# openclimatefix/graph_weather

Measured on AMD Instinct MI355X. Metric: forward forecasts/sec (1° grid, 102→78 feat), higher is better.
Workload: dtype f32; 1 GPU; c2: GraphWeatherForecaster 1deg grid (64800 nodes), 102->78 feat, batch=2 on rank 0, fp32, mesh res 2 (5882 nodes), random-init weights; global_batch=2, parallelism=batch-sharded x1, no collective in forward

## Files before the change

### graph_weather_amd/_lib.py

```python
from __future__ import annotations

import ctypes
import os
import subprocess
from ctypes import POINTER, Structure, c_char_p, c_float, c_int, c_int32, c_int64, c_size_t, c_void_p

_HERE = os.path.dirname(os.path.abspath(__file__))
CSRC = os.path.join(_HERE, "csrc")
LIB_PATH = os.path.join(CSRC, "libgw_amd.so")
HIPCC_FLAGS = ["--offload-arch=gfx950", "-O3", "-std=c++17", "-munsafe-fp-atomics", "-shared", "-fPIC"]

ABI_VERSION = 19
DTYPE_F32, DTYPE_BF16, DTYPE_BF16X3 = 0, 1, 2
LAYOUT_ROWS_F32, LAYOUT_EDGE_TILES_BF16, LAYOUT_ROWS_F16, LAYOUT_ROWS_BF16K = 0, 1, 2, 3
EDGE_DETERMINISTIC, EDGE_SEGMENT_TILES, EDGE_AGG_BF16K, EDGE_SEGMENT_SPLIT = 1, 2, 4, 8

EXPORTS = [
    "gw_version", "gw_last_error", "gw_debug_timestamps", "gw_packed_floats", "gw_pack_linear", "gw_packed_bytes_bf16",
    "gw_pack_linear_bf16", "gw_packed_bytes_bf16x3", "gw_pack_linear_bf16x3", "gw_padded_n", "gw_pad_vector", "gw_pack_many", "gw_mlp_chain_backward", "gw_mlp_chain_backward_bf16x3", "gw_mlp_ln_chain_backward",
    "gw_mlp_forward", "gw_mlp_post_forward", "gw_project_forward", "gw_edge_update_forward", "gw_edge_update_workspace_bytes", "gw_edge_tiles_bytes",
    "gw_edge_rows_to_tiles", "gw_node_update_forward", "gw_node_update_row_split_groups", "gw_node_update_head_forward",
    "gw_normalized_mse_forward", "gw_gemm_f32", "gw_relu_backward", "gw_layernorm_backward", "gw_gather_rows",
    "gw_segment_sum_rows", "gw_normalized_mse_backward", "gw_adamw_step", "gw_nudging_forward", "gw_nudging_backward",
    "gw_linear_forward", "gw_linear_gather_forward", "gw_layernorm_forward", "gw_add_rows", "gw_gather_rows_wide", "gw_segment_sum_rows_wide",
    "gw_constraint_workspace_bytes", "gw_constraint_forward", "gw_constraint_backward",
    "gw_thermal_conv_forward", "gw_thermal_conv_wgrad_workspace_bytes", "gw_thermal_conv_wgrad", "gw_thermal_colsum_workspace_bytes",
    "gw_thermal_colsum", "gw_thermal_groupnorm_workspace_bytes", "gw_thermal_groupnorm_forward", "gw_thermal_groupnorm_backward",
    "gw_thermal_maxpool_forward", "gw_thermal_maxpool_backward", "gw_thermal_resize_forward", "gw_thermal_resize_backward",
    "gw_thermal_rows",
    "gw_amse_mmax", "gw_amse_dft_rows", "gw_amse_legendre_floats", "gw_amse_coeff_floats", "gw_amse_workspace_bytes",
    "gw_amse_forward", "gw_amse_backward",
    "gw_modulate_workspace_bytes", "gw_sdl_forward", "gw_sdl_backward", "gw_film_forward", "gw_film_backward",
    "gw_attention_forward", "gw_attention_backward", "gw_knn_interpolate_forward", "gw_knn_interpolate_backward",
    "gw_gelu_forward", "gw_gelu_backward",
    "gw_attention_axial_forward", "gw_attention_axial_backward",
    "gw_patch_workspace_bytes", "gw_patch_embed_forward", "gw_patch_embed_backward", "gw_patch_expand_forward",
    "gw_patch_expand_backward",
    "gw_attention_masked_forward", "gw_attention_masked_backward",
    "gw_earth_loss_workspace_bytes", "gw_earth_loss_forward", "gw_earth_loss_backward",
    "gw_token_mean_forward", "gw_token_mean_backward", "gw_relu_forward", "gw_row_scale",
    "gw_conv3d_workspace_bytes", "gw_conv3d_forward", "gw_conv3d_backward",
    "gw_gemm_tn_ordered_workspace_bytes", "gw_gemm_tn_ordered", "gw_layernorm_backward_ordered_workspace_bytes",
    "gw_layernorm_backward_ordered",
    "gw_encoder_fused_forward",
    "gw_graph_attention_forward", "gw_graph_attention_backward", "gw_cond_layernorm_forward", "gw_cond_layernorm_backward",
    "gw_beta_gate_forward", "gw_beta_gate_workspace_bytes", "gw_beta_gate_backward", "gw_silu_forward", "gw_silu_backward",
    "gw_fourier_forward", "gw_fourier_backward",
    "gw_graph_attention_batched_forward", "gw_graph_attention_batched_backward", "gw_cond_layernorm_grouped_forward",
    "gw_cond_layernorm_grouped_workspace_bytes", "gw_cond_layernorm_grouped_backward", "gw_gencast_precond_input_forward",
    "gw_gencast_precond_input_backward", "gw_gencast_precond_output_forward", "gw_gencast_precond_output_backward",
    "gw_isht_lmax", "gw_isht_legendre_floats", "gw_isht_workspace_bytes", "gw_isht_forward",
    "gw_gencast_sampler_combine", "gw_gencast_weighted_mse_workspace_bytes", "gw_gencast_weighted_mse_forward",
    "gw_gencast_weighted_mse_backward",
    "gw_cond_layernorm_fanout_forward", "gw_cond_layernorm_fanout_workspace_bytes", "gw_cond_layernorm_fanout_backward",
    "gw_linear_gather_grouped_forward", "gw_segment_sum_rows_grouped",
]

GEMM_NN, GEMM_TN, GEMM_TN_BF16X3 = 0, 1, 2


class GwOperand(Structure):
    _fields_ = [("ptr", c_void_p), ("index", c_void_p), ("rows_per_batch", c_int32), ("ld", c_int32), ("k", c_int32),
                ("projected", c_int32), ("layout", c_int32)]


class GwMlpWeights(Structure):
    _fields_ = [("w1", c_void_p * 3), ("b1", c_void_p), ("w_mid", c_void_p), ("b_mid", c_void_p), ("w_out", c_void_p),
# ... 109 lines not shown
    L.gw_pad_vector.argtypes = [c_void_p, c_int, c_void_p, c_void_p]
    L.gw_mlp_chain_backward.restype = c_int
    L.gw_mlp_chain_backward.argtypes = [c_int64, c_void_p, c_int32, c_int32, POINTER(c_void_p), POINTER(c_void_p), POINTER(c_void_p),
                                        c_int32, POINTER(c_void_p), POINTER(c_void_p), c_void_p]
    L.gw_mlp_chain_backward_bf16x3.restype = c_int
    L.gw_mlp_chain_backward_bf16x3.argtypes = L.gw_mlp_chain_backward.argtypes
    L.gw_mlp_ln_chain_backward.restype = c_int
    L.gw_mlp_ln_chain_backward.argtypes = [c_int32, c_int64, c_void_p, c_int32, c_void_p, c_int32, c_int32, c_void_p, c_int32,
                                           c_void_p, c_void_p, c_void_p, c_void_p, c_void_p,
                                           c_int32, POINTER(c_void_p), POINTER(c_void_p), POINTER(c_void_p), c_void_p,
                                           c_int32, POINTER(c_void_p), POINTER(c_void_p), POINTER(c_void_p), c_int32, ctypes.c_uint32, c_void_p]
    L.gw_pack_many.restype = c_int
    L.gw_pack_many.argtypes = [c_int32, c_int32, POINTER(GwPackItem), c_int32, POINTER(GwPadItem), c_void_p]
    L.gw_mlp_forward.restype = c_int
    L.gw_mlp_forward.argtypes = [c_int64, c_int32, POINTER(GwOperand), POINTER(GwMlpWeights), POINTER(GwOperand),
                                 c_void_p, c_int32, POINTER(GwActivationSave), c_void_p]
    L.gw_mlp_post_forward.restype = c_int
    L.gw_mlp_post_forward.argtypes = [c_int64, c_int32, POINTER(GwOperand), POINTER(GwMlpWeights), c_void_p, c_int32, c_int32,
                                      POINTER(c_void_p), POINTER(c_void_p), c_int32, c_void_p]
    L.gw_edge_update_forward.restype = c_int
    L.gw_edge_update_forward.argtypes = [c_int32, c_int32, c_void_p, c_void_p, POINTER(GwOperand), POINTER(GwOperand),
                                         POINTER(GwOperand), POINTER(GwOperand), POINTER(GwMlpWeights), c_void_p, c_int32, c_void_p,
                                         c_int32, POINTER(GwActivationSave), c_void_p, c_size_t, c_int32, c_void_p]
    L.gw_encoder_fused_forward.restype = c_int
    L.gw_encoder_fused_forward.argtypes = [c_int32, c_int32, c_void_p, c_void_p, POINTER(GwOperand), POINTER(GwMlpWeights),
                                           POINTER(GwOperand), POINTER(GwOperand), POINTER(GwOperand), POINTER(GwMlpWeights), c_void_p,
                                           c_int32, POINTER(GwActivationSave), c_int32, c_void_p]
    L.gw_edge_tiles_bytes.restype = c_size_t
    L.gw_edge_tiles_bytes.argtypes = [c_int32, c_int32]
    L.gw_edge_rows_to_tiles.restype = c_int
    L.gw_edge_rows_to_tiles.argtypes = [c_int32, c_int32, c_void_p, c_int32, c_int32, c_void_p, c_void_p]
    L.gw_edge_update_workspace_bytes.restype = c_size_t
    L.gw_edge_update_workspace_bytes.argtypes = [c_int32, c_int32, POINTER(GwOperand), POINTER(GwOperand), POINTER(GwOperand),
                                                 POINTER(GwMlpWeights), c_int32]
    L.gw_node_update_forward.restype = c_int
    L.gw_node_update_forward.argtypes = [c_int64, c_int32, POINTER(GwOperand), POINTER(GwOperand), POINTER(GwOperand),
                                         POINTER(GwMlpWeights), c_void_p, c_int32, POINTER(GwActivationSave), c_int32,
                                         POINTER(c_void_p), POINTER(c_void_p), c_int32, c_void_p, c_void_p]
    L.gw_node_update_row_split_groups.restype = c_int
    L.gw_node_update_row_split_groups.argtypes = [c_int64]
    L.gw_node_update_head_forward.restype = c_int
    L.gw_node_update_head_forward.argtypes = [c_int64, c_int32, POINTER(GwOperand), POINTER(GwOperand), POINTER(GwMlpWeights),
                                              POINTER(GwMlpWeights), POINTER(GwOperand), c_void_p, c_int32, c_void_p]
    L.gw_project_forward.restype = c_int
    L.gw_project_forward.argtypes = [c_int64, c_int32, POINTER(GwOperand), c_int32, POINTER(c_void_p), POINTER(c_void_p),
                                     c_int32, c_int32, c_int32, c_void_p, c_void_p, c_void_p]
# ... 276 lines not shown
```

### graph_weather_amd/csrc/gw_edge_common.hpp

```cpp
#ifndef GW_EDGE_COMMON_HPP
#define GW_EDGE_COMMON_HPP

#include <hip/hip_runtime.h>
#include <stdint.h>

#include "gw_device.hpp"
#include "gw_internal.hpp"

using namespace gw;

namespace {

constexpr int kStageLd = 260;
constexpr int kStageFloats = kColsPerWG * kStageLd;
constexpr int kEdgeLdsBytes = (kStageFloats + kColsPerWG) * 4;
static_assert(kStageFloats * 4 >= kLdsBytes, "staging area must cover the weight double buffer");
constexpr int kChunkFloats = kChunkSteps * 1024;
constexpr int kChunksPerLayer = 64 / kChunkSteps;

#ifdef GW_TUNING
#define GW_DMA6(a) ((a).dma6)
#else
#define GW_DMA6(a) 0
#endif
// ... 104 lines not shown
        if (s_ == 5) issue_pieces<1>(nsrc_, ((ci + 1) & 1) * kLdsBufFloats, 7, lane, wave);                    \
      } else if ((NEXT_EXISTS) && s_ < kDmaSteps && GW_SKIP(a) != 4) {                                              \
        issue_pieces<8 / kDmaSteps>(nsrc_, ((ci + 1) & 1) * kLdsBufFloats, s_ * (8 / kDmaSteps), lane, wave);  \
      }                                                                                                        \
      if (s_ + 1 < kChunkSteps) {                                                                              \
        _Pragma("unroll") for (int b4 = 0; b4 < 4; ++b4) a_nxt_[b4] = *(const f32x4*)(bl_ + (s_ + 1) * 1024 + b4 * 256); \
      } else if (NEXT_EXISTS) {                                                                                \
        WAIT_STMT;                                                                                             \
        if (GW_SKIP(a) != 5) lds_barrier();                                                                        \
        const float* bn_ = lds + ((ci + 1) & 1) * kLdsBufFloats + lane * 4;                                    \
        _Pragma("unroll") for (int b4 = 0; b4 < 4; ++b4) a_nxt_[b4] = *(const f32x4*)(bn_ + b4 * 256);          \
      }                                                                                                        \
      const float b_ = IN8[s_];                                                                                \
      __builtin_amdgcn_sched_barrier(0);                                                                       \
      _Pragma("unroll") for (int t = 0; t < 16; ++t)                                                           \
          ACC[t] = __builtin_amdgcn_mfma_f32_16x16x4f32(a_cur[t >> 2][t & 3], b_, ACC[t], 0, 0, 0);             \
      __builtin_amdgcn_sched_barrier(0);                                                                       \
      if (s_ + 1 < kChunkSteps || (NEXT_EXISTS)) {                                                             \
        _Pragma("unroll") for (int b4 = 0; b4 < 4; ++b4) a_cur[b4] = a_nxt_[b4];                                \
      }                                                                                                        \
    }                                                                                                          \
    ++ci;                                                                                                      \
  }

#define GW_REQUEST_SLICE(slot, slice)                                          \
  {                                                                            \
    _Pragma("unroll") for (int p = 0; p < NPROJ; ++p) {                        \
      ring[slot][p][0] = hld4<128 * (slice)>(prow[p]);                         \
      ring[slot][p][1] = hld4<128 * (slice) + 64>(prow[p]);                    \
    }                                                                          \
  }

#define GW_TILE_COORDS(N_COLS, N_EDGES, XCD_BASE, XCD_REM)                                \
  const int lane = threadIdx.x & 63;                                                      \
  const int wave = __builtin_amdgcn_readfirstlane(threadIdx.x >> 6);                      \
  const int j = lane & 15;                                                                \
  const int q = lane >> 4;                                                                \
  int tile = blockIdx.x;                                                                  \
  if ((XCD_BASE) > 0) {                                                                   \
    const int xcd = tile & 7, idx = tile >> 3;                                            \
    tile = xcd * (XCD_BASE) + (xcd < (XCD_REM) ? xcd : (XCD_REM)) + idx;                  \
  }                                                                                       \
  const int tile_c0 = tile * kColsPerWG;                                                  \
  const int c_raw = tile_c0 + wave * kColsPerWave + j;                                    \
  const bool valid = c_raw < (N_COLS);                                                    \
  const int c = valid ? c_raw : (N_COLS) - 1;                                             \
  const int b = c / (N_EDGES);                                                            \
  const int k = c - b * (N_EDGES);

__device__ __forceinline__ void stagger_start(int stagger) {
  if (stagger > 0 && (blockIdx.x >> 8) == 1) {
    for (int i = 0; i < stagger; ++i) __builtin_amdgcn_s_sleep(127);
  }
}

constexpr int kConstSetFloats = 5 * 256;
constexpr int kConstOff = kStageFloats + kColsPerWG;
static_assert((kConstOff * 4) % 16 == 0, "constants are read as 16-byte vectors");
constexpr int kB1 = 0, kBMid = 256, kBOut = 512, kGamma = 768, kBeta = 1024;
__device__ __forceinline__ float hld1(const float* p) {
  float v;
  asm volatile("global_load_dword %0, %1, off" : "=v"(v) : "v"(p) : "memory");
  return v;
}
__device__ __forceinline__ void consts_to_lds(float* lds, int set, const float* cv) {
  float* cw = lds + kConstOff + threadIdx.x;
  cw[set + kB1] = cv[0];
  cw[set + kBMid] = cv[1];
  cw[set + kBOut] = cv[2];
  cw[set + kGamma] = cv[3];
  cw[set + kBeta] = cv[4];
}

#define GW_LDS4(p) (*(const f32x4*)(p))
#define GW_LAYERNORM256(O, LD4, GAMMA, BETA, RES)                                                              \
  {                                                                                                            \
    constexpr float inv_n = 1.0f / 256.0f;                                                                     \
    float s = 0.f;                                                                                             \
    _Pragma("unroll") for (int t = 0; t < 16; ++t) s += (O[t].x + O[t].y) + (O[t].z + O[t].w);                 \
    s += __shfl_xor(s, 16);                                                                                    \
    s += __shfl_xor(s, 32);                                                                                    \
    const float mean = s * inv_n;                                                                              \
    float v = 0.f;                                                                                             \
    _Pragma("unroll") for (int t = 0; t < 16; ++t) _Pragma("unroll") for (int r = 0; r < 4; ++r) {             \
      const float d = O[t][r] - mean;                                                                          \
      v += d * d;                                                                                              \
    }                                                                                                          \
// ... 18 lines not shown
  const int* gdl = (const int*)(lds + kStageFloats);

__device__ __forceinline__ void store_e_rows(const float* lds, float* e_out, int tile_c0, int n_cols, int wave, int lane) {
#pragma unroll 4
  for (int i = 0; i < kColsPerWave; ++i) {
    const int col = wave * kColsPerWave + i;
    if (tile_c0 + col < n_cols) {
      const f32x4 vv = *(const f32x4*)(lds + col * kStageLd + 4 * lane);
      stg4(e_out + (size_t)(tile_c0 + col) * 256 + 4 * lane, vv);
    }
  }
}

#define GW_SEGMENT_SUM_ATOMICS(AGG)                                                                            \
  {                                                                                                            \
    const int f = threadIdx.x;                                                                                 \
    float vv[kColsPerWG];                                                                                      \
    _Pragma("unroll") for (int i = 0; i < kColsPerWG; ++i) vv[i] = lds[i * kStageLd + f];                      \
    const int gdv = gdl[lane];                                                                                 \
    const int gdn = gdl[lane < kColsPerWG - 1 ? lane + 1 : lane];                                              \
    const unsigned long long ends = __ballot(lane == kColsPerWG - 1 || gdn != gdv);  \
    float run = 0.f;                                                                                           \
    bool first = true;                                                                                         \
    _Pragma("unroll") for (int i = 0; i < kColsPerWG; ++i) {                                                   \
      run += vv[i];                                                                                            \
      if (__builtin_expect((ends >> i) & 1ull, 0)) {                                                           \
        const int cur = __builtin_amdgcn_readlane(gdv, i);                                                     \
        if (cur >= 0) {                                                                                        \
          float* dstp = (AGG) + (size_t)cur * 256 + f;                                                         \
          if (first || i == kColsPerWG - 1) {                                                                  \
            __hip_atomic_fetch_add((GW_AS1 float*)dstp, run, __ATOMIC_RELAXED, __HIP_MEMORY_SCOPE_AGENT);      \
          } else {                                                                                             \
            stg1(dstp, run);                                                                                   \
          }                                                                                                    \
        }                                                                                                      \
        first = false;                                                                                         \
        run = 0.f;                                                                                             \
      }                                                                                                        \
    }                                                                                                          \
  }

template <typename K, typename A>
int launch_tile_kernel(K kernel, const A& a, int lds_bytes, const char* name, void* stream) {
  static DeviceOnce once;
  if (once.first()) (void)hipFuncSetAttribute((const void*)kernel, hipFuncAttributeMaxDynamicSharedMemorySize, lds_bytes);
  const int grid = (a.n_cols + kColsPerWG - 1) / kColsPerWG;
  hipLaunchKernelGGL(kernel, dim3(grid), dim3(kThreads), lds_bytes, (hipStream_t)stream, a);
  return check_launch(name);
// ... 27 lines not shown
```

### graph_weather_amd/csrc/gw_edge_lds.hip

```cpp

#include <hip/hip_runtime.h>
#include <stdint.h>
#include <string.h>

#include "gw_device.hpp"
#include "gw_edge_common.hpp"
#include "gw_internal.hpp"

using namespace gw;

namespace {

constexpr int kEldsLdsBytes = (kConstOff + kConstSetFloats) * 4;
static_assert(kEldsLdsBytes == 71936, "staging + destination ids + one set of constants");
static_assert(2 * kEldsLdsBytes <= 160 * 1024, "two workgroups per CU must fit the 160 KiB of LDS");

struct EldsArgs {
  int n_cols;
  int n_edges;
  int n_dst;
  int stagger;
  int skip;
  int dma6;
  int xcd_base;
// ... 13 lines not shown
  const float* w_mid;
  const float* b_mid;
  const float* w_out;
  const float* b_out;
  const float* gamma;
  const float* beta;
  const float* res_ptr;
  int res_rows_pb;
  int res_ld;
  float* e_out;
  float* agg;
};

template <bool RAW>
__device__ __forceinline__ const float* chunk_src(const EldsArgs& a, int i) {
  if (RAW) {
    if (i < kChunksPerLayer) return a.w_raw + (size_t)i * kChunkFloats;
    i -= kChunksPerLayer;
  }
  if (i < kChunksPerLayer) return a.w_mid + (size_t)i * kChunkFloats;
  return a.w_out + (size_t)(i - kChunksPerLayer) * kChunkFloats;
}

template <int N>
__device__ __forceinline__ void wait_prologue(int& s, int& d, float (&c)[5]) {
  asm volatile("s_waitcnt vmcnt(%[n])" : "+v"(s), "+v"(d), "+v"(c[0]), "+v"(c[1]), "+v"(c[2]), "+v"(c[3]), "+v"(c[4]) : [n] "n"(N) : "memory");
}

template <bool RAW, int NPROJ>
__global__ __launch_bounds__(kThreads, 2) void elds_kernel(const EldsArgs a) {
  float* const lds = lds_base();
  const float* const cst = lds + kConstOff;
  GW_TILE_COORDS(a.n_cols, a.n_edges, a.xcd_base, a.xcd_rem)
  stagger_start(a.stagger);

  int s_idx = hldi(a.src + k);
  int d_idx = hldi(a.dst + k);
  float cv[5];
  {
    const int f = threadIdx.x;
    cv[0] = hld1(a.b1 + f);
    cv[1] = hld1(a.b_mid + f);
    cv[2] = hld1(a.b_out + f);
    cv[3] = hld1(a.gamma + f);
    cv[4] = hld1(a.beta + f);
  }
  issue_chunk32k(chunk_src<RAW>(a, 0), lds, lane, wave);
  int ci = 0;
  wait_prologue<8>(s_idx, d_idx, cv);
  consts_to_lds(lds, 0, cv);

// ... 239 lines not shown
```

### graph_weather_amd/csrc/gw_edge_stream.hip

```cpp

#include <hip/hip_runtime.h>
#include <stdint.h>
#include <string.h>

#include "gw_device.hpp"
#include "gw_edge_common.hpp"
#include "gw_internal.hpp"

using namespace gw;

namespace {

constexpr int kStreamLdsBytes = (kConstOff + kConstSetFloats) * 4;
static_assert(2 * kStreamLdsBytes <= 160 * 1024, "two workgroups per CU must fit the 160 KiB of LDS");

struct StreamArgs {
  int n_cols;
  int n_edges;
  int n_dst;
  int stagger;
  int skip;
  int dma6;
  int xcd_base;
  int xcd_rem;
  const int* src;
  const int* dst;
  const float* p_ptr[2];
  int p_rows_pb[2];
  int p_ld[2];
  int p_kind[2];
  const float* b1;
  const float* w_mid;
  const float* b_mid;
  const float* w_out;
  const float* b_out;
  const float* gamma;
  const float* beta;
  float* agg;
};

__device__ __forceinline__ const float* chunk_src(const StreamArgs& a, int i) {
  if (i < kChunksPerLayer) return a.w_mid + (size_t)i * kChunkFloats;
  return a.w_out + (size_t)(i - kChunksPerLayer) * kChunkFloats;
}

template <int NPROJ>
__global__ __launch_bounds__(kThreads, 2) void estream_kernel(const StreamArgs a) {
  float* const lds = lds_base();
  const float* const cst = lds + kConstOff;
  GW_TILE_COORDS(a.n_cols, a.n_edges, a.xcd_base, a.xcd_rem)
  stagger_start(a.stagger);

  int s_idx = hldi(a.src + k);
  int d_idx = hldi(a.dst + k);
  issue_chunk32k(chunk_src(a, 0), lds, lane, wave);
  int ci = 0;
  {
    const int f = threadIdx.x;
    const float cv[5] = {ldg1(a.b1 + f), ldg1(a.b_mid + f), ldg1(a.b_out + f), ldg1(a.gamma + f), ldg1(a.beta + f)};
    consts_to_lds(lds, 0, cv);
  }
  wait_regs<0>(s_idx, d_idx);

  const float* prow[NPROJ];
#pragma unroll
  for (int p = 0; p < NPROJ; ++p) {
    const int r = a.p_kind[p] == 0 ? s_idx : (a.p_kind[p] == 1 ? d_idx : k);
    prow[p] = a.p_ptr[p] + ((size_t)b * (size_t)a.p_rows_pb[p] + (size_t)r) * (size_t)a.p_ld[p] + 4 * q;
  }
  const int gd_id = valid ? b * a.n_dst + d_idx : -1;

  f32x4 ring[2][NPROJ][2];
#define GW_BIAS_SLICE(slice)                                                   \
  {                                                                            \
    bb0 = *(const f32x4*)(cst + kB1 + 32 * (slice) + 4 * q);                   \
    bb1 = *(const f32x4*)(cst + kB1 + 32 * (slice) + 16 + 4 * q);              \
  }
#define GW_CONSUME_SLICE(slot, slice)                                          \
  {                                                                            \
    f32x4 v0_ = ring[slot][0][0], v1_ = ring[slot][0][1];                      \
    _Pragma("unroll") for (int p = 1; p < NPROJ; ++p) {                        \
      v0_ += ring[slot][p][0];                                                 \
      v1_ += ring[slot][p][1];                                                 \
    }                                                                          \
    v0_ += bb0;                                                                \
    v1_ += bb1;                                                                \
    _Pragma("unroll") for (int r = 0; r < 4; ++r) {                            \
      in8[r] = fmaxf(v0_[r], 0.f);                                             \
      in8[4 + r] = fmaxf(v1_[r], 0.f);                                         \
    }                                                                          \
  }

  f32x4 a_cur[4];
  f32x4 acc2[16];
  float in8[8];
  f32x4 bb0, bb1;
  GW_REQUEST_SLICE(0, 0)
  GW_REQUEST_SLICE(1, 1)
  wait_regs<2 * NPROJ>(ring[0]);
  lds_barrier();
#pragma unroll
  for (int t = 0; t < 16; ++t) acc2[t] = *(const f32x4*)(cst + kBMid + 16 * t + 4 * q);
  GW_BIAS_SLICE(0)
#pragma unroll
  for (int b4 = 0; b4 < 4; ++b4) a_cur[b4] = *(const f32x4*)(lds + lane * 4 + b4 * 256);
  GW_CONSUME_SLICE(0, 0)
  GW_REQUEST_SLICE(0, 2)

#define GW_PRODUCE_CHUNK(cc)                                                              \
  {                                                                                       \
    if ((cc) + 1 < kChunksPerLayer) GW_BIAS_SLICE((cc) + 1)                                \
    if ((cc) <= 6) {                                                                      \
      GW_CHUNK(acc2, in8, true, wait_regs<0>(ring[((cc) + 1) & 1]), chunk_src(a, ci + 1))                        \
    } else {                                                                              \
      GW_CHUNK(acc2, in8, true, wait_vm<0>(), chunk_src(a, ci + 1))                                              \
    }                                                                                     \
    if ((cc) + 1 < kChunksPerLayer) GW_CONSUME_SLICE(((cc) + 1) & 1, (cc) + 1)             \
  }
  GW_PRODUCE_CHUNK(0)
  GW_REQUEST_SLICE(1, 3)
  GW_PRODUCE_CHUNK(1)
  GW_REQUEST_SLICE(0, 4)
  GW_PRODUCE_CHUNK(2)
  GW_REQUEST_SLICE(1, 5)
  GW_PRODUCE_CHUNK(3)
  GW_REQUEST_SLICE(0, 6)
  GW_PRODUCE_CHUNK(4)
  GW_REQUEST_SLICE(1, 7)
  GW_PRODUCE_CHUNK(5)
  GW_PRODUCE_CHUNK(6)
  GW_PRODUCE_CHUNK(7)

  float hin[64];
#pragma unroll
  for (int t = 0; t < 16; ++t)
#pragma unroll
    for (int r = 0; r < 4; ++r) hin[4 * t + r] = fmaxf(acc2[t][r], 0.f);
  f32x4 o[16];
#pragma unroll
  for (int t = 0; t < 16; ++t) o[t] = f32x4{0.f, 0.f, 0.f, 0.f};
#pragma unroll
  for (int cc = 0; cc < kChunksPerLayer; ++cc) {
#pragma unroll
    for (int i = 0; i < 8; ++i) in8[i] = hin[8 * cc + i];
    if (cc + 1 < kChunksPerLayer) {
      GW_CHUNK(o, in8, true, wait_vm<0>(), chunk_src(a, ci + 1))
    } else {
      GW_CHUNK(o, in8, false, wait_vm<0>(), chunk_src(a, ci + 1))
    }
  }

#pragma unroll
  for (int t = 0; t < 16; ++t) o[t] += *(const f32x4*)(cst + kBOut + 16 * t + 4 * q);
  GW_LAYERNORM256(o, GW_LDS4, cst + kGamma, cst + kBeta, )
  GW_STAGE_ROWS(o, gd_id)
  GW_SEGMENT_SUM_ATOMICS(a.agg)
#undef GW_BIAS_SLICE
#undef GW_CONSUME_SLICE
#undef GW_PRODUCE_CHUNK
}

inline bool is_proj_f32(const gw_operand* op) { return op->k > 0 && op->projected && op->layout == GW_LAYOUT_ROWS_F32; }

}

namespace gw {

bool edge_stream_eligible(const gw_operand* x_src, const gw_operand* x_dst, const gw_operand* e_in, const gw_mlp_weights* w) {
  if (w->weight_dtype != GW_DTYPE_F32 || w->n_mid != 1 || !w->ln_gamma || !w->ln_beta || !w->w_mid || !w->b_mid) return false;
  if (w->ln_width > 0 && w->ln_width != 256) return false;
  const gw_operand* ops[3] = {x_src, x_dst, e_in};
  int n_proj = 0;
  for (int i = 0; i < 3; ++i) {
    if (ops[i]->k == 0) continue;
    if (!is_proj_f32(ops[i])) return false;
    ++n_proj;
  }
  return n_proj == 1 || n_proj == 2;
}

int edge_stream_launch(int32_t batch, int32_t n_edges, const int32_t* src, const int32_t* dst, const gw_operand* x_src,
                       const gw_operand* x_dst, const gw_operand* e_in, const gw_mlp_weights* w, float* agg, int32_t n_dst,
// ... 7 lines not shown
  a.src = src;
  a.dst = dst;
  const gw_operand* ops[3] = {x_src, x_dst, e_in};
  int n_proj = 0;
  for (int i = 0; i < 3; ++i) {
    if (ops[i]->k == 0) continue;
    if (n_proj == 2) return set_error(GW_E_UNSUPPORTED, "edge_stream_launch: at most two projected operands");
    a.p_ptr[n_proj] = ops[i]->ptr;
    a.p_rows_pb[n_proj] = ops[i]->rows_per_batch;
    a.p_ld[n_proj] = ops[i]->ld;
    a.p_kind[n_proj] = i;
    ++n_proj;
  }
  if (n_proj == 0) return set_error(GW_E_UNSUPPORTED, "edge_stream_launch: no projected operand");
  a.b1 = w->b1;
  a.w_mid = w->w_mid;
  a.b_mid = w->b_mid;
  a.w_out = w->w_out;
  a.b_out = w->b_out;
  a.gamma = w->ln_gamma;
  a.beta = w->ln_beta;
  a.agg = agg;
  fill_tile_schedule(a, tiles, 2);
  if (a.skip != 4 && a.skip != 5) a.skip = 0;
  const char* what = "estream_kernel launch";
  return n_proj == 1 ? launch_tile_kernel(estream_kernel<1>, a, kStreamLdsBytes, what, stream)
                     : launch_tile_kernel(estream_kernel<2>, a, kStreamLdsBytes, what, stream);
}

}
```

### graph_weather_amd/csrc/gw_encoder_fused.hip

```cpp

#include <hip/hip_runtime.h>
#include <stdint.h>
#include <string.h>

#include "gw_device.hpp"
#include "gw_edge_common.hpp"
#include "gw_internal.hpp"

using namespace gw;

namespace {

constexpr int kNodeSteps = 28;
constexpr int kNodeSet = 0, kEdgeSet = kConstSetFloats;
constexpr int kEncfLdsBytes = (kConstOff + 2 * kConstSetFloats) * 4;
static_assert(kEncfLdsBytes == 77056, "staging (66 560) + destination ids (256) + constants (10 240)");
static_assert(2 * kEncfLdsBytes <= 160 * 1024, "two workgroups per CU must fit the 160 KiB of LDS");

struct EncfArgs {
  int n_cols;
  int n_edges;
  int n_dst;
  int stagger;
  int xcd_base;
// ... 42 lines not shown
               : "+v"(c[0]), "+v"(c[1]), "+v"(c[2]), "+v"(c[3]), "+v"(c[4]), "+v"(c[5]), "+v"(c[6]), "+v"(c[7]), "+v"(c[8]), "+v"(c[9])
               :
               : "memory");
}
__device__ __forceinline__ void wait_pairs(f32x2 (&r)[14]) {
  asm volatile("s_waitcnt vmcnt(0)"
               : "+v"(r[0]), "+v"(r[1]), "+v"(r[2]), "+v"(r[3]), "+v"(r[4]), "+v"(r[5]), "+v"(r[6]), "+v"(r[7]), "+v"(r[8]), "+v"(r[9]),
                 "+v"(r[10]), "+v"(r[11]), "+v"(r[12]), "+v"(r[13])
               :
               : "memory");
}
__device__ __forceinline__ void wait_singles(float (&r)[kNodeSteps]) {
  asm volatile("s_waitcnt vmcnt(0)"
               : "+v"(r[0]), "+v"(r[1]), "+v"(r[2]), "+v"(r[3]), "+v"(r[4]), "+v"(r[5]), "+v"(r[6]), "+v"(r[7]), "+v"(r[8]), "+v"(r[9]),
                 "+v"(r[10]), "+v"(r[11]), "+v"(r[12]), "+v"(r[13])
               :
               : "memory");
  asm volatile("s_waitcnt vmcnt(0)"
               : "+v"(r[14]), "+v"(r[15]), "+v"(r[16]), "+v"(r[17]), "+v"(r[18]), "+v"(r[19]), "+v"(r[20]), "+v"(r[21]), "+v"(r[22]),
                 "+v"(r[23]), "+v"(r[24]), "+v"(r[25]), "+v"(r[26]), "+v"(r[27])
               :
               : "memory");
}

#define GW_FCHUNK(ACC, IN, OFF, NS, NP, DS, WAIT_STMT)                                                          \
  {                                                                                                            \
    const float* bl_ = lds + (ci & 1) * kLdsBufFloats + lane * 4;                                              \
    const float* nsrc_ = chunk_src(a, (NP) > 0 ? ci + 1 : ci);                                                 \
    _Pragma("unroll") for (int s_ = 0; s_ < (NS); ++s_) {                                                      \
      f32x4 a_nxt_[4];                                                                                         \
      if ((NP) > 0 && s_ < (DS))                                                                               \
        issue_pieces<((NP) > 0 ? (NP) / (DS) : 1)>(nsrc_, ((ci + 1) & 1) * kLdsBufFloats, s_ * ((NP) / (DS)), lane, wave); \
      if (s_ + 1 < (NS)) {                                                                                     \
        _Pragma("unroll") for (int b4 = 0; b4 < 4; ++b4) a_nxt_[b4] = *(const f32x4*)(bl_ + (s_ + 1) * 1024 + b4 * 256); \
      } else if ((NP) > 0) {                                                                                   \
        WAIT_STMT;                                                                                             \
        lds_barrier();                                                                                         \
        const float* bn_ = lds + ((ci + 1) & 1) * kLdsBufFloats + lane * 4;                                    \
        _Pragma("unroll") for (int b4 = 0; b4 < 4; ++b4) a_nxt_[b4] = *(const f32x4*)(bn_ + b4 * 256);          \
      }                                                                                                        \
      const float b_ = IN[(OFF) + s_];                                                                         \
      __builtin_amdgcn_sched_barrier(0);                                                                       \
      _Pragma("unroll") for (int t = 0; t < 16; ++t)                                                           \
          ACC[t] = __builtin_amdgcn_mfma_f32_16x16x4f32(a_cur[t >> 2][t & 3], b_, ACC[t], 0, 0, 0);             \
      __builtin_amdgcn_sched_barrier(0);                                                                       \
      if (s_ + 1 < (NS) || (NP) > 0) {                                                                         \
        _Pragma("unroll") for (int b4 = 0; b4 < 4; ++b4) a_cur[b4] = a_nxt_[b4];                                \
      }                                                                                                        \
    }                                                                                                          \
    ++ci;                                                                                                      \
  }

template <bool RES, int NPROJ>
__global__ __launch_bounds__(kThreads, 2) void encfused_kernel(const EncfArgs a) {
  float* const lds = lds_base();
  const float* const cst = lds + kConstOff;
  GW_TILE_COORDS(a.n_cols, a.n_edges, a.xcd_base, a.xcd_rem)
  stagger_start(a.stagger);

  int s_idx = hldi(a.src + k);
  int d_idx = hldi(a.dst + k);
  float cv[10];
  {
    const int f = threadIdx.x;
#pragma unroll
    for (int i = 0; i < 5; ++i) cv[i] = hld1(a.n_const[i] + f);
#pragma unroll
    for (int i = 0; i < 5; ++i) cv[5 + i] = hld1(a.e_const[i] + f);
  }
  issue_chunk32k(chunk_src(a, 0), lds, lane, wave);
  int ci = 0;
  wait_regs<18>(s_idx, d_idx);
  const float* prow[NPROJ];
#pragma unroll
// ... 287 lines not shown
```

### include/gw_amd.h

```cpp
#ifndef GW_AMD_H
#define GW_AMD_H

#include <stddef.h>
#include <stdint.h>

#ifdef __cplusplus
extern "C" {
#endif

#define GW_OK 0
#define GW_E_BADARG (-1)
#define GW_E_UNSUPPORTED (-2)
#define GW_E_LAUNCH (-3)

#define GW_ABI_VERSION 19

#define GW_DTYPE_F32 0
#define GW_DTYPE_BF16 1
#define GW_DTYPE_BF16X3 2

#define GW_LAYOUT_ROWS_F32 0
#define GW_LAYOUT_EDGE_TILES_BF16 1
#define GW_LAYOUT_ROWS_F16 2
#define GW_LAYOUT_ROWS_BF16K 3
// ... 101 lines not shown
                           void* e_out ,
                           int32_t e_out_layout , float* agg ,
                           int32_t n_dst, const struct gw_activation_save* save ,
                           void* workspace , size_t workspace_bytes, int32_t flags , void* stream);
size_t gw_edge_tiles_bytes(int32_t batch, int32_t n_edges);
int gw_edge_rows_to_tiles(int32_t batch, int32_t n_edges, const float* rows, int32_t rows_per_batch, int32_t ld, void* tiles,
                          void* stream);
size_t gw_edge_update_workspace_bytes(int32_t batch, int32_t n_edges, const gw_operand* x_src, const gw_operand* x_dst,
                                      const gw_operand* e_in, const gw_mlp_weights* w, int32_t flags);

int gw_encoder_fused_forward(int32_t batch, int32_t n_edges, const int32_t* src, const int32_t* dst, const gw_operand* features,
                             const gw_mlp_weights* w_node, const gw_operand* x_dst, const gw_operand* e_in, const gw_operand* e_res,
                             const gw_mlp_weights* w_edge, float* agg , int32_t n_dst,
                             const struct gw_activation_save* save , int32_t flags , void* stream);

int gw_node_update_forward(int64_t n_rows, int32_t rows_per_batch, const gw_operand* x, const gw_operand* x_res,
                           const gw_operand* agg, const gw_mlp_weights* w, float* x_out, int32_t out_ld,
                           const struct gw_activation_save* save ,
                           int32_t n_post , const float* const* post_w, void* const* post_out,
                           int32_t post_layout ,
                           float* zero_rows , void* stream);

int gw_node_update_row_split_groups(int64_t n_rows);

int gw_node_update_head_forward(int64_t n_rows, int32_t rows_per_batch, const gw_operand* x, const gw_operand* agg,
                                const gw_mlp_weights* w, const gw_mlp_weights* head, const gw_operand* residual ,
                                float* out, int32_t out_ld, void* stream);

int gw_normalized_mse_forward(const float* pred, const float* target,
                              const float* inv_var ,
                              int32_t inv_var_full, const float* lat_weights, int32_t num_unique_lat, int32_t batch, int32_t nodes,
                              int32_t channels, float* loss_out, void* stream);


typedef struct gw_activation_save {
  float* hidden;
  int64_t hidden_stride;
  int32_t hidden_ld;
  float* pre_norm;
} gw_activation_save;

#define GW_GEMM_NN 0
#define GW_GEMM_TN 1
#define GW_GEMM_TN_BF16X3 2
int gw_gemm_f32(int32_t mode, int64_t m, int32_t n, int64_t k, const float* a, int32_t lda, const float* b, int32_t ldb,
                float* c, int32_t ldc, float* colsum_a ,
// ... 304 lines not shown
```

Before: 314.3 forecasts/s.

## Shrink edge-stream LDS footprint to fit three workgroups per CU

The edge-stream MLP kernel moves from two large double-buffered weight chunks to a ring of smaller 4-step chunks with counted waits. The output stage now writes half a tile at a time and keeps destination ids in LDS. Together these cut LDS use to about 38 KB, so launch bounds can allow three workgroups per CU instead of two, aiming at more latency hiding. The cost is more barriers and more chunk handovers, plus added register pressure under the higher occupancy bound; an occupancy query export is also added.

```diff
diff --git a/graph_weather_amd/_lib.py b/graph_weather_amd/_lib.py
--- a/graph_weather_amd/_lib.py
+++ b/graph_weather_amd/_lib.py
@@ -42,7 +42,7 @@
     "gw_conv3d_workspace_bytes", "gw_conv3d_forward", "gw_conv3d_backward",
     "gw_gemm_tn_ordered_workspace_bytes", "gw_gemm_tn_ordered", "gw_layernorm_backward_ordered_workspace_bytes",
     "gw_layernorm_backward_ordered",
-    "gw_encoder_fused_forward",
+    "gw_encoder_fused_forward", "gw_edge_stream_workgroups_per_cu",
     "gw_graph_attention_forward", "gw_graph_attention_backward", "gw_cond_layernorm_forward", "gw_cond_layernorm_backward",
     "gw_beta_gate_forward", "gw_beta_gate_workspace_bytes", "gw_beta_gate_backward", "gw_silu_forward", "gw_silu_backward",
     "gw_fourier_forward", "gw_fourier_backward",
@@ -198,6 +198,8 @@
     L.gw_edge_update_forward.argtypes = [c_int32, c_int32, c_void_p, c_void_p, POINTER(GwOperand), POINTER(GwOperand),
                                          POINTER(GwOperand), POINTER(GwOperand), POINTER(GwMlpWeights), c_void_p, c_int32, c_void_p,
                                          c_int32, POINTER(GwActivationSave), c_void_p, c_size_t, c_int32, c_void_p]
+    L.gw_edge_stream_workgroups_per_cu.restype = c_int
+    L.gw_edge_stream_workgroups_per_cu.argtypes = [c_int]
     L.gw_encoder_fused_forward.restype = c_int
     L.gw_encoder_fused_forward.argtypes = [c_int32, c_int32, c_void_p, c_void_p, POINTER(GwOperand), POINTER(GwMlpWeights),
                                            POINTER(GwOperand), POINTER(GwOperand), POINTER(GwOperand), POINTER(GwMlpWeights), c_void_p,
diff --git a/graph_weather_amd/csrc/gw_edge_common.hpp b/graph_weather_amd/csrc/gw_edge_common.hpp
--- a/graph_weather_amd/csrc/gw_edge_common.hpp
+++ b/graph_weather_amd/csrc/gw_edge_common.hpp
@@ -150,6 +150,41 @@
     }                                                                                                          \
     ++ci;                                                                                                      \
   }
+
+#define GW_RCHUNK(ACC, IN, OFF, NS, NP, DS, HANDOVER, WAIT_STMT, MID_STMT, CUR_BUF, NEXT_BUF, DMA_BUF, DMA_SRC)       \
+  {                                                                                                            \
+    const float* bl_ = lds + (CUR_BUF) + lane * 4;                                                             \
+    const float* nsrc_ = (DMA_SRC);                                                                            \
+    _Pragma("unroll") for (int s_ = 0; s_ < (NS); ++s_) {                                                      \
+      f32x4 a_nxt_[4];                                                                                         \
+      if ((NP) > 0 && s_ < (DS))                                                                               \
+        issue_pieces<((NP) > 0 ? (NP) / (DS) : 1)>(nsrc_, (DMA_BUF), s_ * ((NP) / (DS)), lane, wave);          \
+      if (s_ == (DS)) {                                                                                        \
+        MID_STMT;                                                                                              \
+      }                                                                                                        \
+      if (s_ + 1 < (NS)) {                                                                                     \
+        _Pragma("unroll") for (int b4 = 0; b4 < 4; ++b4) a_nxt_[b4] = *(const f32x4*)(bl_ + (s_ + 1) * 1024 + b4 * 256); \
+      } else if (HANDOVER) {                                                                                   \
+        WAIT_STMT;                                                                                             \
+        lds_barrier();                                                                                         \
+        const float* bn_ = lds + (NEXT_BUF) + lane * 4;                                                        \
+        _Pragma("unroll") for (int b4 = 0; b4 < 4; ++b4) a_nxt_[b4] = *(const f32x4*)(bn_ + b4 * 256);          \
+      }                                                                                                        \
+      const float b_ = IN[(OFF) + s_];                                                                         \
+      __builtin_amdgcn_sched_barrier(0);                                                                       \
+      _Pragma("unroll") for (int t = 0; t < 16; ++t)                                                           \
+          ACC[t] = __builtin_amdgcn_mfma_f32_16x16x4f32(a_cur[t >> 2][t & 3], b_, ACC[t], 0, 0, 0);             \
+      __builtin_amdgcn_sched_barrier(0);                                                                       \
+      if (s_ + 1 < (NS) || (HANDOVER)) {                                                                       \
+        _Pragma("unroll") for (int b4 = 0; b4 < 4; ++b4) a_cur[b4] = a_nxt_[b4];                                \
+      }                                                                                                        \
+    }                                                                                                          \
+    ++ci;                                                                                                      \
+  }
+
+#define GW_FCHUNK(ACC, IN, OFF, NS, NP, DS, WAIT_STMT)                                                          \
+  GW_RCHUNK(ACC, IN, OFF, NS, NP, DS, (NP) > 0, WAIT_STMT, , (ci & 1) * kLdsBufFloats, ((ci + 1) & 1) * kLdsBufFloats,  \
+            ((ci + 1) & 1) * kLdsBufFloats, chunk_src(a, (NP) > 0 ? ci + 1 : ci))
 
 #define GW_REQUEST_SLICE(slot, slice)                                          \
   {                                                                            \
@@ -191,6 +226,10 @@
   asm volatile("global_load_dword %0, %1, off" : "=v"(v) : "v"(p) : "memory");
   return v;
 }
+template <int N>
+__device__ __forceinline__ void wait_prologue(int& s, int& d, float (&c)[5]) {
+  asm volatile("s_waitcnt vmcnt(%[n])" : "+v"(s), "+v"(d), "+v"(c[0]), "+v"(c[1]), "+v"(c[2]), "+v"(c[3]), "+v"(c[4]) : [n] "n"(N) : "memory");
+}
 __device__ __forceinline__ void consts_to_lds(float* lds, int set, const float* cv) {
   float* cw = lds + kConstOff + threadIdx.x;
   cw[set + kB1] = cv[0];
@@ -255,8 +294,13 @@
     const unsigned long long ends = __ballot(lane == kColsPerWG - 1 || gdn != gdv);  \
     float run = 0.f;                                                                                           \
     bool first = true;                                                                                         \
-    _Pragma("unroll") for (int i = 0; i < kColsPerWG; ++i) {                                                   \
-      run += vv[i];                                                                                            \
+    GW_SEGMENT_WALK(AGG, vv, 0, kColsPerWG)                                                                    \
+  }
+
+#define GW_SEGMENT_WALK(AGG, VV, C0, NC)                                                                       \
+  {                                                                                                            \
+    _Pragma("unroll") for (int i = (C0); i < (C0) + (NC); ++i) {                                               \
+      run += VV[i - (C0)];                                                                                     \
       if (__builtin_expect((ends >> i) & 1ull, 0)) {                                                           \
         const int cur = __builtin_amdgcn_readlane(gdv, i);                                                     \
         if (cur >= 0) {                                                                                        \
diff --git a/graph_weather_amd/csrc/gw_edge_lds.hip b/graph_weather_amd/csrc/gw_edge_lds.hip
--- a/graph_weather_amd/csrc/gw_edge_lds.hip
+++ b/graph_weather_amd/csrc/gw_edge_lds.hip
@@ -59,11 +59,6 @@
   return a.w_out + (size_t)(i - kChunksPerLayer) * kChunkFloats;
 }
 
-template <int N>
-__device__ __forceinline__ void wait_prologue(int& s, int& d, float (&c)[5]) {
-  asm volatile("s_waitcnt vmcnt(%[n])" : "+v"(s), "+v"(d), "+v"(c[0]), "+v"(c[1]), "+v"(c[2]), "+v"(c[3]), "+v"(c[4]) : [n] "n"(N) : "memory");
-}
-
 template <bool RAW, int NPROJ>
 __global__ __launch_bounds__(kThreads, 2) void elds_kernel(const EldsArgs a) {
   float* const lds = lds_base();
diff --git a/graph_weather_amd/csrc/gw_edge_stream.hip b/graph_weather_amd/csrc/gw_edge_stream.hip
--- a/graph_weather_amd/csrc/gw_edge_stream.hip
+++ b/graph_weather_amd/csrc/gw_edge_stream.hip
@@ -11,16 +11,33 @@
 
 namespace {
 
-constexpr int kStreamLdsBytes = (kConstOff + kConstSetFloats) * 4;
-static_assert(2 * kStreamLdsBytes <= 160 * 1024, "two workgroups per CU must fit the 160 KiB of LDS");
+#ifndef GW_ESTREAM_RING
+#define GW_ESTREAM_RING 2
+#endif
+constexpr int kSRing = GW_ESTREAM_RING;
+constexpr int kSAhead = kSRing - 1;
+static_assert(kSRing == 2 || kSRing == 3, "the counted waits below are derived for one or two chunks of look-ahead");
+constexpr int kSSteps = 4;
+constexpr int kSPieces = 4;
+constexpr int kSBufFloats = kSSteps * 1024;
+constexpr int kSChunksPerLayer = 64 / kSSteps;
+constexpr int kSHalfCols = kColsPerWG / 2;
+constexpr int kSStageFloats = kSHalfCols * kStageLd;
+constexpr int kSIdsOff = kSRing * kSBufFloats > kSStageFloats ? kSRing * kSBufFloats : kSStageFloats;
+constexpr int kSConstOff = kSIdsOff + kColsPerWG;
+constexpr int kSSet = kSConstOff - kConstOff;
+constexpr int kStreamLdsBytes = (kSConstOff + kConstSetFloats) * 4;
+#if GW_ESTREAM_RING == 2
+static_assert(kStreamLdsBytes == 38656, "staging of a half tile over the ring (33 280) + destination ids (256) + constants (5 120)");
+#endif
+static_assert((kSConstOff * 4) % 16 == 0, "constants are read as 16-byte vectors");
+static_assert(3 * kStreamLdsBytes <= 160 * 1024, "three workgroups per CU must fit the 160 KiB of LDS");
 
 struct StreamArgs {
   int n_cols;
   int n_edges;
   int n_dst;
   int stagger;
-  int skip;
-  int dma6;
   int xcd_base;
   int xcd_rem;
   const int* src;
@@ -40,27 +57,44 @@
 };
 
 __device__ __forceinline__ const float* chunk_src(const StreamArgs& a, int i) {
-  if (i < kChunksPerLayer) return a.w_mid + (size_t)i * kChunkFloats;
-  return a.w_out + (size_t)(i - kChunksPerLayer) * kChunkFloats;
-}
+  if (i < kSChunksPerLayer) return a.w_mid + (size_t)i * kSBufFloats;
+  return a.w_out + (size_t)(i - kSChunksPerLayer) * kSBufFloats;
+}
+
+__device__ __forceinline__ void pin_regs(f32x4 (&r)[16]) {
+  asm volatile(""
+               : "+v"(r[0]), "+v"(r[1]), "+v"(r[2]), "+v"(r[3]), "+v"(r[4]), "+v"(r[5]), "+v"(r[6]), "+v"(r[7]), "+v"(r[8]),
+                 "+v"(r[9]), "+v"(r[10]), "+v"(r[11]), "+v"(r[12]), "+v"(r[13]), "+v"(r[14]), "+v"(r[15]));
+}
+
+#define GW_SCHUNK(ACC, IN, OFF, NP, HANDOVER, WAIT_STMT, MID_STMT)                                              \
+  GW_RCHUNK(ACC, IN, OFF, kSSteps, NP, 2, HANDOVER, WAIT_STMT, MID_STMT, (ci % kSRing) * kSBufFloats,          \
+            ((ci + 1) % kSRing) * kSBufFloats, ((ci + kSAhead) % kSRing) * kSBufFloats,                        \
+            chunk_src(a, (NP) > 0 ? ci + kSAhead : ci))
 
 template <int NPROJ>
-__global__ __launch_bounds__(kThreads, 2) void estream_kernel(const StreamArgs a) {
+__global__ __launch_bounds__(kThreads, 3) void estream_kernel(const StreamArgs a) {
   float* const lds = lds_base();
-  const float* const cst = lds + kConstOff;
+  const float* const cst = lds + kSConstOff;
   GW_TILE_COORDS(a.n_cols, a.n_edges, a.xcd_base, a.xcd_rem)
   stagger_start(a.stagger);
 
   int s_idx = hldi(a.src + k);
   int d_idx = hldi(a.dst + k);
-  issue_chunk32k(chunk_src(a, 0), lds, lane, wave);
-  int ci = 0;
+  float cv[5];
   {
     const int f = threadIdx.x;
-    const float cv[5] = {ldg1(a.b1 + f), ldg1(a.b_mid + f), ldg1(a.b_out + f), ldg1(a.gamma + f), ldg1(a.beta + f)};
-    consts_to_lds(lds, 0, cv);
-  }
-  wait_regs<0>(s_idx, d_idx);
+    cv[0] = hld1(a.b1 + f);
+    cv[1] = hld1(a.b_mid + f);
+    cv[2] = hld1(a.b_out + f);
+    cv[3] = hld1(a.gamma + f);
+    cv[4] = hld1(a.beta + f);
+  }
+  issue_pieces<kSPieces>(chunk_src(a, 0), 0, 0, lane, wave);
+  if (kSAhead == 2) issue_pieces<kSPieces>(chunk_src(a, 1), kSBufFloats, 0, lane, wave);
+  int ci = 0;
+  wait_prologue<kSPieces * kSAhead>(s_idx, d_idx, cv);
+  consts_to_lds(lds, kSSet, cv);
 
   const float* prow[NPROJ];
 #pragma unroll
@@ -68,7 +102,7 @@
     const int r = a.p_kind[p] == 0 ? s_idx : (a.p_kind[p] == 1 ? d_idx : k);
     prow[p] = a.p_ptr[p] + ((size_t)b * (size_t)a.p_rows_pb[p] + (size_t)r) * (size_t)a.p_ld[p] + 4 * q;
   }
-  const int gd_id = valid ? b * a.n_dst + d_idx : -1;
+  if (q == 0) ((int*)(lds + kSIdsOff))[wave * kColsPerWave + j] = valid ? b * a.n_dst + d_idx : -1;
 
   f32x4 ring[2][NPROJ][2];
 #define GW_BIAS_SLICE(slice)                                                   \
@@ -105,31 +139,30 @@
 #pragma unroll
   for (int b4 = 0; b4 < 4; ++b4) a_cur[b4] = *(const f32x4*)(lds + lane * 4 + b4 * 256);
   GW_CONSUME_SLICE(0, 0)
-  GW_REQUEST_SLICE(0, 2)
-
-#define GW_PRODUCE_CHUNK(cc)                                                              \
-  {                                                                                       \
-    if ((cc) + 1 < kChunksPerLayer) GW_BIAS_SLICE((cc) + 1)                                \
-    if ((cc) <= 6) {                                                                      \
-      GW_CHUNK(acc2, in8, true, wait_regs<0>(ring[((cc) + 1) & 1]), chunk_src(a, ci + 1))                        \
-    } else {                                                                              \
-      GW_CHUNK(acc2, in8, true, wait_vm<0>(), chunk_src(a, ci + 1))                                              \
-    }                                                                                     \
-    if ((cc) + 1 < kChunksPerLayer) GW_CONSUME_SLICE(((cc) + 1) & 1, (cc) + 1)             \
-  }
-  GW_PRODUCE_CHUNK(0)
-  GW_REQUEST_SLICE(1, 3)
-  GW_PRODUCE_CHUNK(1)
-  GW_REQUEST_SLICE(0, 4)
-  GW_PRODUCE_CHUNK(2)
-  GW_REQUEST_SLICE(1, 5)
-  GW_PRODUCE_CHUNK(3)
-  GW_REQUEST_SLICE(0, 6)
-  GW_PRODUCE_CHUNK(4)
-  GW_REQUEST_SLICE(1, 7)
-  GW_PRODUCE_CHUNK(5)
-  GW_PRODUCE_CHUNK(6)
-  GW_PRODUCE_CHUNK(7)
+
+#define GW_PRODUCE_PAIR(cc)                                                                                            \
+  {                                                                                                                    \
+    if ((cc) + 1 < 8) GW_BIAS_SLICE((cc) + 1)                                                                           \
+    if ((cc) <= 5) {                                                                                                   \
+      GW_SCHUNK(acc2, in8, 0, kSPieces, true, wait_vm<2 * NPROJ + 4 * (kSAhead - 1)>(), GW_REQUEST_SLICE((cc) & 1, (cc) + 2)) \
+      GW_SCHUNK(acc2, in8, 4, kSPieces, true, wait_regs<(kSAhead - 1) * (2 * NPROJ + 4)>(ring[((cc) + 1) & 1]), )      \
+    } else if ((cc) == 6) {                                                                                            \
+      GW_SCHUNK(acc2, in8, 0, kSPieces, true, wait_vm<4 * (kSAhead - 1)>(), )                                           \
+      GW_SCHUNK(acc2, in8, 4, kSPieces, true, wait_regs<4 * (kSAhead - 1)>(ring[1]), )                                  \
+    } else {                                                                                                           \
+      GW_SCHUNK(acc2, in8, 0, kSPieces, true, wait_vm<4 * (kSAhead - 1)>(), )                                           \
+      GW_SCHUNK(acc2, in8, 4, kSPieces, true, wait_vm<4 * (kSAhead - 1)>(), )                                           \
+    }                                                                                                                  \
+    if ((cc) + 1 < 8) GW_CONSUME_SLICE(((cc) + 1) & 1, (cc) + 1)                                                        \
+  }
+  GW_PRODUCE_PAIR(0)
+  GW_PRODUCE_PAIR(1)
+  GW_PRODUCE_PAIR(2)
+  GW_PRODUCE_PAIR(3)
+  GW_PRODUCE_PAIR(4)
+  GW_PRODUCE_PAIR(5)
+  GW_PRODUCE_PAIR(6)
+  GW_PRODUCE_PAIR(7)
 
   float hin[64];
 #pragma unroll
@@ -140,24 +173,52 @@
 #pragma unroll
   for (int t = 0; t < 16; ++t) o[t] = f32x4{0.f, 0.f, 0.f, 0.f};
 #pragma unroll
-  for (int cc = 0; cc < kChunksPerLayer; ++cc) {
-#pragma unroll
-    for (int i = 0; i < 8; ++i) in8[i] = hin[8 * cc + i];
-    if (cc + 1 < kChunksPerLayer) {
-      GW_CHUNK(o, in8, true, wait_vm<0>(), chunk_src(a, ci + 1))
+  for (int cc = 0; cc < kSChunksPerLayer; ++cc) {
+    if (cc + kSAhead < kSChunksPerLayer) {
+      GW_SCHUNK(o, hin, kSSteps * cc, kSPieces, true, wait_vm<4 * (kSAhead - 1)>(), )
+    } else if (cc + 1 < kSChunksPerLayer) {
+      GW_SCHUNK(o, hin, kSSteps * cc, 0, true, wait_vm<0>(), )
     } else {
-      GW_CHUNK(o, in8, false, wait_vm<0>(), chunk_src(a, ci + 1))
+      GW_SCHUNK(o, hin, kSSteps * cc, 0, false, wait_vm<0>(), )
     }
   }
 
 #pragma unroll
   for (int t = 0; t < 16; ++t) o[t] += *(const f32x4*)(cst + kBOut + 16 * t + 4 * q);
   GW_LAYERNORM256(o, GW_LDS4, cst + kGamma, cst + kBeta, )
-  GW_STAGE_ROWS(o, gd_id)
-  GW_SEGMENT_SUM_ATOMICS(a.agg)
+  pin_regs(o);
+#define GW_STAGE_HALF(O)                                                                   \
+  {                                                                                        \
+    float* srow = lds + ((wave & 1) * kColsPerWave + (lane_e & 15)) * kStageLd + 4 * (lane_e >> 4); \
+    _Pragma("unroll") for (int t = 0; t < 16; ++t) *(f32x4*)(srow + 16 * t) = O[t];        \
+  }
+  const int* const gdl = (const int*)(lds + kSIdsOff);
+  const int lane_e = __builtin_amdgcn_mbcnt_hi(~0u, __builtin_amdgcn_mbcnt_lo(~0u, 0u));
+  __syncthreads();
+  if (wave < 2) GW_STAGE_HALF(o)
+  __syncthreads();
+  {
+    const int f = threadIdx.x;
+    const int gdv = gdl[lane];
+    const int gdn = gdl[lane < kColsPerWG - 1 ? lane + 1 : lane];
+    const unsigned long long ends = __ballot(lane == kColsPerWG - 1 || gdn != gdv);
+    float run = 0.f;
+    bool first = true;
+    float vv[kSHalfCols];
+#pragma unroll
+    for (int i = 0; i < kSHalfCols; ++i) vv[i] = lds[i * kStageLd + f];
+    GW_SEGMENT_WALK(a.agg, vv, 0, kSHalfCols)
+    lds_barrier();
+    if (wave >= 2) GW_STAGE_HALF(o)
+    lds_barrier();
+#pragma unroll
+    for (int i = 0; i < kSHalfCols; ++i) vv[i] = lds[i * kStageLd + f];
+    GW_SEGMENT_WALK(a.agg, vv, kSHalfCols, kSHalfCols)
+  }
+#undef GW_STAGE_HALF
 #undef GW_BIAS_SLICE
 #undef GW_CONSUME_SLICE
-#undef GW_PRODUCE_CHUNK
+#undef GW_PRODUCE_PAIR
 }
 
 inline bool is_proj_f32(const gw_operand* op) { return op->k > 0 && op->projected && op->layout == GW_LAYOUT_ROWS_F32; }
@@ -211,10 +272,22 @@
   a.beta = w->ln_beta;
   a.agg = agg;
   fill_tile_schedule(a, tiles, 2);
-  if (a.skip != 4 && a.skip != 5) a.skip = 0;
   const char* what = "estream_kernel launch";
   return n_proj == 1 ? launch_tile_kernel(estream_kernel<1>, a, kStreamLdsBytes, what, stream)
                      : launch_tile_kernel(estream_kernel<2>, a, kStreamLdsBytes, what, stream);
 }
 
-}
+int edge_stream_workgroups_per_cu(int n_proj) {
+  if (n_proj != 1 && n_proj != 2) return set_error(GW_E_UNSUPPORTED, "edge_stream_workgroups_per_cu: one or two projected operands");
+  const void* kernel = n_proj == 1 ? (const void*)estream_kernel<1> : (const void*)estream_kernel<2>;
+  if (hipFuncSetAttribute(kernel, hipFuncAttributeMaxDynamicSharedMemorySize, kStreamLdsBytes) != hipSuccess)
+    return set_error(GW_E_LAUNCH, "edge_stream_workgroups_per_cu: hipFuncSetAttribute");
+  int n = 0;
+  if (hipOccupancyMaxActiveBlocksPerMultiprocessor(&n, kernel, kThreads, (size_t)kStreamLdsBytes) != hipSuccess)
+    return set_error(GW_E_LAUNCH, "edge_stream_workgroups_per_cu: hipOccupancyMaxActiveBlocksPerMultiprocessor");
+  return n;
+}
+
+}
+
+extern "C" int gw_edge_stream_workgroups_per_cu(int n_proj) { return gw::edge_stream_workgroups_per_cu(n_proj); }
diff --git a/graph_weather_amd/csrc/gw_encoder_fused.hip b/graph_weather_amd/csrc/gw_encoder_fused.hip
--- a/graph_weather_amd/csrc/gw_encoder_fused.hip
+++ b/graph_weather_amd/csrc/gw_encoder_fused.hip
@@ -88,34 +88,6 @@
                :
                : "memory");
 }
-
-#define GW_FCHUNK(ACC, IN, OFF, NS, NP, DS, WAIT_STMT)                                                          \
-  {                                                                                                            \
-    const float* bl_ = lds + (ci & 1) * kLdsBufFloats + lane * 4;                                              \
-    const float* nsrc_ = chunk_src(a, (NP) > 0 ? ci + 1 : ci);                                                 \
-    _Pragma("unroll") for (int s_ = 0; s_ < (NS); ++s_) {                                                      \
-      f32x4 a_nxt_[4];                                                                                         \
-      if ((NP) > 0 && s_ < (DS))                                                                               \
-        issue_pieces<((NP) > 0 ? (NP) / (DS) : 1)>(nsrc_, ((ci + 1) & 1) * kLdsBufFloats, s_ * ((NP) / (DS)), lane, wave); \
-      if (s_ + 1 < (NS)) {                                                                                     \
-        _Pragma("unroll") for (int b4 = 0; b4 < 4; ++b4) a_nxt_[b4] = *(const f32x4*)(bl_ + (s_ + 1) * 1024 + b4 * 256); \
-      } else if ((NP) > 0) {                                                                                   \
-        WAIT_STMT;                                                                                             \
-        lds_barrier();                                                                                         \
-        const float* bn_ = lds + ((ci + 1) & 1) * kLdsBufFloats + lane * 4;                                    \
-        _Pragma("unroll") for (int b4 = 0; b4 < 4; ++b4) a_nxt_[b4] = *(const f32x4*)(bn_ + b4 * 256);          \
-      }                                                                                                        \
-      const float b_ = IN[(OFF) + s_];                                                                         \
-      __builtin_amdgcn_sched_barrier(0);                                                                       \
-      _Pragma("unroll") for (int t = 0; t < 16; ++t)                                                           \
-          ACC[t] = __builtin_amdgcn_mfma_f32_16x16x4f32(a_cur[t >> 2][t & 3], b_, ACC[t], 0, 0, 0);             \
-      __builtin_amdgcn_sched_barrier(0);                                                                       \
-      if (s_ + 1 < (NS) || (NP) > 0) {                                                                         \
-        _Pragma("unroll") for (int b4 = 0; b4 < 4; ++b4) a_cur[b4] = a_nxt_[b4];                                \
-      }                                                                                                        \
-    }                                                                                                          \
-    ++ci;                                                                                                      \
-  }
 
 template <bool RES, int NPROJ>
 __global__ __launch_bounds__(kThreads, 2) void encfused_kernel(const EncfArgs a) {
diff --git a/include/gw_amd.h b/include/gw_amd.h
--- a/include/gw_amd.h
+++ b/include/gw_amd.h
@@ -147,6 +147,8 @@
                            float* zero_rows , void* stream);
 
 int gw_node_update_row_split_groups(int64_t n_rows);
+
+int gw_edge_stream_workgroups_per_cu(int n_proj);
 
 int gw_node_update_head_forward(int64_t n_rows, int32_t rows_per_batch, const gw_operand* x, const gw_operand* agg,
                                 const gw_mlp_weights* w, const gw_mlp_weights* head, const gw_operand* residual ,
```

Result: no change. 316.8 forecasts/s, median of 6 (+0.8%).
